# kirumang/Pix2Pose

Measured on AMD Instinct MI355X. Metric: crops/sec (AE fwd + PnP-RANSAC) at 128x128, higher is better.
Workload: dtype f16x3 (fp32 operands split into two f16 halves, 3 MFMAs per product block, fp32 accumulate)

## Files before the change

### pix2pose_amd/build.py

```python
from __future__ import annotations

import hashlib
import os
import subprocess

HERE = os.path.dirname(os.path.abspath(__file__))
CSRC = os.path.join(HERE, "csrc")
LIB = os.path.join(HERE, "libp2p_mi355.so")
DEV_LIB = os.path.join(HERE, "libp2p_mi355_dev.so")
DEV_OBJ_DIR = os.path.join(CSRC, "dev")
SOURCES = ["igemm.hip", "igemm_halo.hip", "igemm_halo8.hip", "igemm_halo_s2.hip", "igemm_stream.hip", "wino.hip", "wino3.hip", "wino3o.hip", "resblock.hip", "heads.hip", "conv1.hip", "misc_kernels.hip", "model.hip", "pipeline.hip", "resize_aa.hip", "pnp.hip", "comm.hip", "depth.hip", "normals.hip", "icp.hip", "rgbd.hip", "xyz_patch.hip", "train_batch.hip"]
HEADERS = ["kernels.h", "device_common.h", "igemm_halo_common.h", "wino_common.h", "model.h", "pipeline.h", "resize_rules.h", os.path.join("..", "..", "include", "p2p_mi355.h")]
BUILD_ID_SRC = os.path.join(CSRC, "_build_id.cpp")
EXPORT_MAP = os.path.join(CSRC, "_exports.map")
HIPCC = os.environ.get("HIPCC", "/opt/rocm/bin/hipcc")
FLAGS = ["--offload-arch=gfx950", "-O3", "-std=c++17", "-fPIC", "-fvisibility=hidden", "-Wall", "-Wno-unused-function", "-Wno-unused-value", "-Wno-unused-result"]


def _newer(a: str, b: str) -> bool:
    return not os.path.exists(b) or os.path.getmtime(a) > os.path.getmtime(b)


def _files():
    srcs = [os.path.join(CSRC, s) for s in SOURCES if os.path.exists(os.path.join(CSRC, s))]
# ... 20 lines not shown


def _compile_and_link(lib: str, obj_dir: str, extra_flags, force: bool, verbose: bool) -> str:
    srcs, hdrs = _files()
    os.makedirs(obj_dir, exist_ok=True)
    objs = []
    hdr_time = max(os.path.getmtime(h) for h in hdrs)
    procs = []
    for s in srcs:
        o = os.path.join(obj_dir, os.path.splitext(os.path.basename(s))[0] + ".o")
        objs.append(o)
        if force or _newer(s, o) or os.path.getmtime(o) < hdr_time:
            cmd = [HIPCC] + FLAGS + list(extra_flags) + ["-c", s, "-o", o]
            if verbose:
                print(" ".join(cmd))
            procs.append((cmd, subprocess.Popen(cmd)))
            if len(procs) >= JOBS:
                c, pr = procs.pop(0)
                if pr.wait():
                    raise subprocess.CalledProcessError(pr.returncode, c)
    for c, pr in procs:
        if pr.wait():
            raise subprocess.CalledProcessError(pr.returncode, c)
    bid = source_hash()
    text = '// generated by pix2pose_amd/build.py\nextern "C" __attribute__((visibility("default"))) const char* p2p_build_id(void) { return "%s"; }\n' % bid
    if not os.path.exists(BUILD_ID_SRC) or open(BUILD_ID_SRC).read() != text:
        open(BUILD_ID_SRC, "w").write(text)
    bo = os.path.join(obj_dir, "_build_id.o")
    if force or _newer(BUILD_ID_SRC, bo):
        subprocess.check_call(["g++", "-O1", "-fPIC", "-fvisibility=hidden", "-c", BUILD_ID_SRC, "-o", bo])
    objs.append(bo)
    import re
    names = sorted(set(re.findall(r"\bP2P_API\s+[\w\s\*]+?\b(p2p_[a-z0-9_]+)\s*\(", open(os.path.join(HERE, "..", "include", "p2p_mi355.h")).read())))
    vtext = "{ global: %s; local: *; };\n" % "; ".join(names)
    if not os.path.exists(EXPORT_MAP) or open(EXPORT_MAP).read() != vtext:
        open(EXPORT_MAP, "w").write(vtext)
    if force or any(_newer(o, lib) for o in objs) or _newer(EXPORT_MAP, lib):
        cmd = [HIPCC, "--offload-arch=gfx950", "-shared", "-fPIC", "-Wl,--version-script=" + EXPORT_MAP, "-o", lib] + objs + ["-ldl"]
        if verbose:
            print(" ".join(cmd))
        subprocess.check_call(cmd)
    return lib


JOBS = max(1, min(4, (os.cpu_count() or 2) // 2))


def build(force: bool = False, verbose: bool = False, dev: bool = True) -> str:
    lib = _compile_and_link(LIB, CSRC, [], force, verbose)
    if dev:
        _compile_and_link(DEV_LIB, DEV_OBJ_DIR, ["-DP2P_DEV_SWITCHES"], force, verbose)
    return lib


def dev_switches(**switches) -> dict:
    override = os.environ.get("P2P_DEV_LIB")
    if override:
        if not os.path.exists(override):
            raise RuntimeError("P2P_DEV_LIB=%s does not exist" % override)
        env = {"P2P_LIB": override}
        env.update({k: str(v) for k, v in switches.items()})
        return env
    if have_sources() and have_compiler():
        _compile_and_link(DEV_LIB, DEV_OBJ_DIR, ["-DP2P_DEV_SWITCHES"], False, False)
    elif not os.path.exists(DEV_LIB):
        raise RuntimeError("development twin %s is missing and cannot be built here" % DEV_LIB)
# ... 9 lines not shown
```

### pix2pose_amd/csrc/kernels.h

```cpp
#pragma once
#include <hip/hip_runtime.h>
#include <stdint.h>
#include <stdlib.h>

namespace p2p {

#ifdef P2P_DEV_SWITCHES
inline const char* dev_env(const char* name) { return getenv(name); }
#else
inline const char* dev_env(const char*) { return nullptr; }
#endif

struct Ctx;
extern thread_local Ctx* g_prof_ctx;
struct ProfScope {
    Ctx* ctx;
    hipStream_t s;
    int slot;
    double flops, bytes;
    hipEvent_t a = nullptr, b = nullptr;
    bool failed = false;
    ProfScope(Ctx* X, int slot_, hipStream_t st, double fl = 0.0, double by = 0.0) : ctx(X), s(st), slot(slot_), flops(fl), bytes(by) { if (ctx) open(); }
    ProfScope(int slot_, hipStream_t st) : ProfScope(g_prof_ctx, slot_, st) {}
    ~ProfScope() { if (ctx) (void)close(); }
// ... 111 lines not shown
    int n_groups;
    ResBlockGroup grp[IGEMM_MAX_GROUPS + 1];
};
bool resblock_supported(int F1, int H, int W);
int resblock_grid(int F1, int N, int H, int W);
hipError_t launch_resblock(const ResBlockParams& p, int F1, hipStream_t s);
hipError_t launch_resproj(const ResBlockParams& p, int F1, hipStream_t s);

struct WinoGroup {
    const float* U;
    const float* scale;
    const float* shift;
    int sample0;
    int unit0;
};
struct WinoParams {
    IgemmSeg seg[2];
    unsigned seg_bytes[2];
    int seg0_groups;
    int N, H, W, Cin, Cout;
    float* V;
    const float* U;
    const float* scale;
    const float* shift;
    int act;
    float alpha;
    float* out;
    int out_cstride, out_coff;
    unsigned* range_acc;
    int n_groups;
    WinoGroup grp[IGEMM_MAX_GROUPS + 1];
    int ksplit;
    float* partial;
};
bool wino_supported(int H, int W, int Cin0, int Cin1, int Cout);
size_t wino_v_bytes(int N, int H, int W, int Cin);
int wino_gemm_grid(const WinoParams& p);
hipError_t launch_wino_input(const WinoParams& p, hipStream_t s);
hipError_t launch_wino_gemm(const WinoParams& p, int n_cu, hipStream_t s);

struct Wino3Params {
    const float* in;
    unsigned in_bytes;
    int N, H, W, Cin, Cout;
    float* V;
    const float* U;
    const float* scale;
    const float* shift;
    int act;
    float alpha;
    float* out;
    int out_cstride, out_coff;
    unsigned* range_acc;
    int n_groups;
    WinoGroup grp[IGEMM_MAX_GROUPS + 1];
};
bool wino3_supported(int H, int W, int Cin, int Cout);
size_t wino3_v_bytes(int N, int H, int W, int Cin);
hipError_t launch_wino3_input(const Wino3Params& p, hipStream_t s);
hipError_t launch_wino3_gemm(const Wino3Params& p, int n_cu, hipStream_t s);

struct Wino3oParams {
    const float* in;
    unsigned in_bytes;
    int N, Cin, Cout;
    float* V;
    const float* U;
    const float* scale;
    const float* shift;
    int act;
    float alpha;
    float* out;
    int out_cstride, out_coff;
    int ksplit;
    float* partial;
    unsigned* range_acc;
    int n_groups;
    WinoGroup grp[IGEMM_MAX_GROUPS + 1];
};
bool wino3o_supported(int mode, int Cin, int Cout);
size_t wino3o_v_bytes(int mode, int units, int Cin);
int wino3o_units(const Wino3oParams& p);
hipError_t launch_wino3o_input(const Wino3oParams& p, int mode, hipStream_t s);
hipError_t launch_wino3o_gemm(const Wino3oParams& p, int mode, int n_cu, hipStream_t s);

struct StreamOrder {
    int n_groups;
    int8_t gstart[IGEMM_MAX_TAPS + 3];
// ... 52 lines not shown
```

### pix2pose_amd/csrc/model.hip

```cpp
#include "model.h"

#include <cmath>
#include <cstdarg>
#include <cstdio>
#include <cstring>
#include <thread>

namespace p2p {

static thread_local char g_err[512] = "";

void set_error(const char* fmt, ...)
{
    va_list ap;
    va_start(ap, fmt);
    vsnprintf(g_err, sizeof(g_err), fmt, ap);
    va_end(ap);
}
const char* get_error() { return g_err; }

constexpr double BN_EPS = 1e-3;
constexpr float LEAKY = 0.3f;

struct TensorMap {
// ... 950 lines not shown
        static const int max_s2 = dev_env("P2P_SMALL_SPLIT_S2") ? atoi(dev_env("P2P_SMALL_SPLIT_S2")) : 256;
        int S = tiles <= (c.in_stride == 2 ? max_s2 : max_s1) ? std::min(std::min(16, 768 / std::max(1, tiles)), p.ksteps / 12) : 1;
        while (S >= 2 && (size_t)S * p.M * L.Cout > (size_t)X.max_batch * 64 * 64 * 128 * 2) --S;
        if (S >= 2) {
            ConvCall c2 = c;
            c2.ksplit = S; c2.partial = X.cur->act["wv"];
            PreparedConv pc2;
            if ((rc = prepare_conv(X, L, c2, pc2))) return rc;
            if (pc2.stream) {
                if ((rc = launch_prepared(X, &pc2, 1))) return rc;
                HIP_TRY(launch_splitk_reduce(c2.partial, S, p.M, L.Cout, L.scale, L.shift, c.act, LEAKY, c.out, L.prec == PREC_F16X3 ? X.range_cur : nullptr, X.cur->stream));
                return P2P_OK;
            }
        }
    }
    return launch_prepared(X, &pc, 1);
}

static int conv_layer(Ctx& X, const ConvLayer& L, const float* in, int N, int H, int W, int C, int stride,
                      float* out, int act, const float* residual = nullptr)
{
    ConvCall c;
    c.s0 = {in, C, C, 0};
    c.N = N; c.Hin = H; c.Win = W; c.Hg = H / stride; c.Wg = W / stride; c.in_stride = stride;
    c.out = out; c.Hout = c.Hg; c.Wout = c.Wg; c.out_cstride = L.Cout;
    c.act = act; c.residual = residual; c.res_cstride = L.Cout;
    return L.ntaps == 25 ? run_conv_small(X, L, c) : run_conv(X, L, c);
}

constexpr int WINO_MIN_INPUTS = 1;

static bool wino_split_route() { static const bool on = dev_env("P2P_NO_WINO_SPLIT") == nullptr; return on; }

static int try_wino(Ctx& X, const ConvLayer& L, const float* a, int Ca, const float* b, int Cb, int cb_stride, int cb_off, int N, int H, float* out)
{
    if (!L.wino_u || L.prec != PREC_F16X3 || X.wino_mode == P2P_WINOGRAD_OFF || !specialised_kernels() || !wino_supported(H, H, Ca, Cb, L.Cout)) return 0;
    WinoParams p;
    memset(&p, 0, sizeof(p));
    p.seg[0] = {a, Ca, Ca, 0};
    p.seg[1] = {b, Cb, cb_stride, cb_off};
    const size_t px = (size_t)N * H * H;
    const size_t b0 = px * Ca * sizeof(float), b1 = px * cb_stride * sizeof(float);
    if (b0 >= 0xFFFFFFF0ull || b1 >= 0xFFFFFFF0ull || L.wino_bytes >= 0xFFFFFFF0ull) return 0;
    p.seg_bytes[0] = (unsigned)b0; p.seg_bytes[1] = (unsigned)b1;
    p.seg0_groups = Ca / 32;
    p.N = N; p.H = H; p.W = H; p.Cin = Ca + Cb; p.Cout = L.Cout;
    p.V = X.cur->act["wv"];
    p.U = L.wino_u; p.scale = L.wino_scale; p.shift = L.shift;
    p.act = ACT_LEAKY; p.alpha = LEAKY;
    p.out = out; p.out_cstride = L.Cout; p.out_coff = 0;
    p.range_acc = X.range_cur;
    int rc = wino_groups(X, L, 2, "try_wino", p.grp, p.n_groups);
    if (rc) return rc;
    static const int wino_min = dev_env("P2P_WINO_MIN") ? atoi(dev_env("P2P_WINO_MIN")) : WINO_MIN_INPUTS;
    if (X.wino_mode != P2P_WINOGRAD_ALWAYS && N < wino_min) return 0;
    if (X.wino_mode == P2P_WINOGRAD_AUTO && p.n_groups <= 1 && wino_split_route()) {
        const int tiles = wino_gemm_grid(p), S = p.Cin / 16;
        for (int k : {6, 4, 3, 2})
            if (tiles * k <= 256 && S % (2 * k) == 0 && (size_t)k * px * L.Cout <= WINO_PARTIAL_FLOATS) { p.ksplit = k; p.partial = X.cur->act["wp"]; break; }
    }
    hipStream_t st = X.cur->stream;
    const double in_el = (double)px * p.Cin, out_el = (double)px * L.Cout;
    if ((rc = prof_launch(X, 11, 0.0, 4.0 * in_el + 8.0 * in_el, [&]() { return launch_wino_input(p, st); }))) return rc;
    if ((rc = prof_launch(X, 10, 2.0 * out_el * 25.0 * p.Cin, 8.0 * in_el + (double)L.wino_bytes + 4.0 * out_el,
                          [&]() { return launch_wino_gemm(p, X.n_cu, st); }))) return rc;
    if (p.ksplit > 1) HIP_TRY(launch_splitk_reduce(p.partial, p.ksplit, (int)px, L.Cout, L.wino_scale, L.shift, ACT_LEAKY, LEAKY, out, X.range_cur, st));
    return 1;
}

static int concat_conv(Ctx& X, const ConvLayer& L, const float* a, int Ca, const float* b, int Cb,
                       int cb_stride, int cb_off, int N, int H, float* out)
{
    {
        const int rc = try_wino(X, L, a, Ca, b, Cb, cb_stride, cb_off, N, H, out);
        if (rc < 0) return rc;
        if (rc == 1) return P2P_OK;
    }
    ConvCall c;
    c.s0 = {a, Ca, Ca, 0};
    c.s1 = {b, Cb, cb_stride, cb_off};
    c.N = N; c.Hin = H; c.Win = H; c.Hg = H; c.Wg = H;
    c.out = out; c.Hout = H; c.Wout = H; c.out_cstride = L.Cout;
    c.act = ACT_LEAKY;
    return run_conv_small(X, L, c);
}

constexpr int WINO3_MIN_INPUTS = 5;
constexpr int WINO3O_MIN_INPUTS = 9;
static bool wino3_route() { static const bool on = dev_env("P2P_NO_WINO3") == nullptr; return on; }

static int try_wino3o(Ctx& X, const ConvLayer& L, int mode, const float* in, int N, int C, float* out)
{
    if (!L.wino_u || L.prec != PREC_F16X3 || X.wino_mode == P2P_WINOGRAD_OFF || !specialised_kernels() || !wino3_route() || !wino3o_supported(mode, C, L.Cout)) return 0;
    static const int wino3o_min = dev_env("P2P_WINO3O_MIN") ? atoi(dev_env("P2P_WINO3O_MIN")) : WINO3O_MIN_INPUTS;
    if (X.wino_mode != P2P_WINOGRAD_ALWAYS && N < wino3o_min) return 0;
    const size_t b0 = (size_t)N * (mode ? 256 : 64) * C * sizeof(float);
    if (b0 >= 0xFFFFFFF0ull || L.wino_bytes >= 0xFFFFFFF0ull) return 0;
    Wino3oParams p;
    memset(&p, 0, sizeof(p));
    p.in = in; p.in_bytes = (unsigned)b0;
    p.N = N; p.Cin = C; p.Cout = L.Cout;
    p.V = X.cur->act["wv"];
    p.U = L.wino_u; p.scale = L.wino_scale; p.shift = L.shift;
    p.act = ACT_LEAKY; p.alpha = LEAKY;
    p.out = out; p.out_cstride = L.Cout; p.out_coff = 0;
    p.ksplit = 1;
    p.range_acc = X.range_cur;
    int rc = wino_groups(X, L, 8, "try_wino3o", p.grp, p.n_groups);
    if (rc) return rc;
    const int units = wino3o_units(p);
    if (wino3o_v_bytes(mode, units, C) > (size_t)X.max_batch * 64 * 64 * 128 * 2 * sizeof(float)) return 0;
    if (mode == 1 && (X.wino_mode == P2P_WINOGRAD_ALWAYS || units * (L.Cout / 64) < 256)) { p.ksplit = 4; p.partial = X.cur->act["c3"]; }
    hipStream_t st = X.cur->stream;
    const double in_el = (double)N * (mode ? 256 : 64) * C, out_el = (double)N * (mode ? 64 : 256) * L.Cout;
    if ((rc = prof_launch(X, 21, 0.0, 4.0 * in_el + 6.0 * in_el, [&]() { return launch_wino3o_input(p, mode, st); }))) return rc;
    if ((rc = prof_launch(X, 20, 2.0 * out_el * (mode ? 25.0 : 6.25) * C, 6.0 * in_el + (double)L.wino_bytes + 4.0 * out_el,
                          [&]() { return launch_wino3o_gemm(p, mode, X.n_cu, st); }))) return rc;
    if (p.ksplit > 1 && p.n_groups > 1) {
        Conv1Groups G;
        if ((rc = conv1_groups(X, L, N, 64, true, G))) return rc;
        HIP_TRY(launch_splitk_reduce_groups(p.partial, p.ksplit, N * 64, L.Cout, G, ACT_LEAKY, LEAKY, out, X.range_cur, st));
    } else if (p.ksplit > 1)
        HIP_TRY(launch_splitk_reduce(p.partial, p.ksplit, N * 64, L.Cout, L.wino_scale, L.shift, ACT_LEAKY, LEAKY, out, X.range_cur, st));
    return 1;
}

static int try_wino3(Ctx& X, const ConvLayer& L, const float* in, int N, int H, int C, float* out)
{
    if (H == 8) return try_wino3o(X, L, 0, in, N, C, out);
    if (!L.wino_u || L.prec != PREC_F16X3 || X.wino_mode == P2P_WINOGRAD_OFF || !specialised_kernels() || !wino3_route() || !wino3_supported(H, H, C, L.Cout)) return 0;
    static const int wino3_min = dev_env("P2P_WINO3_MIN") ? atoi(dev_env("P2P_WINO3_MIN")) : WINO3_MIN_INPUTS;
    if (X.wino_mode != P2P_WINOGRAD_ALWAYS && N < wino3_min) return 0;
    const size_t px = (size_t)N * H * H;
    const size_t b0 = px * C * sizeof(float);
    if (b0 >= 0xFFFFFFF0ull || L.wino_bytes >= 0xFFFFFFF0ull) return 0;
    Wino3Params p;
    memset(&p, 0, sizeof(p));
    p.in = in; p.in_bytes = (unsigned)b0;
    p.N = N; p.H = H; p.W = H; p.Cin = C; p.Cout = L.Cout;
    p.V = X.cur->act["wv"];
    p.U = L.wino_u; p.scale = L.wino_scale; p.shift = L.shift;
    p.act = ACT_LEAKY; p.alpha = LEAKY;
    p.out = out; p.out_cstride = L.Cout; p.out_coff = 0;
    p.range_acc = X.range_cur;
    int rc = wino_groups(X, L, 2, "try_wino3", p.grp, p.n_groups);
    if (rc) return rc;
    hipStream_t st = X.cur->stream;
    const double in_el = (double)px * C, out_el = 4.0 * (double)px * L.Cout;
    if ((rc = prof_launch(X, 21, 0.0, 4.0 * in_el + 6.0 * in_el, [&]() { return launch_wino3_input(p, st); }))) return rc;
    rc = prof_launch(X, 20, 2.0 * out_el * 6.25 * C, 6.0 * in_el + (double)L.wino_bytes + 4.0 * out_el, [&]() { return launch_wino3_gemm(p, X.n_cu, st); });
    return rc ? rc : 1;
}

static int deconv_layer(Ctx& X, const Model& M, const char* name, const float* in, int N, int H, int C,
                        float* out)
{
    {
        const int rc = try_wino3(X, M.L.at(std::string(name) + "_p0"), in, N, H, C, out);
        if (rc < 0) return rc;
        if (rc == 1) return P2P_OK;
    }
    PreparedConv pc[4];
    bool all_stream = true;
    for (int ph = 0; ph < 4; ++ph) {
        const ConvLayer& L = M.L.at(std::string(name) + "_p" + std::to_string(ph));
        ConvCall c;
        c.s0 = {in, C, C, 0};
        c.N = N; c.Hin = H; c.Win = H; c.Hg = H; c.Wg = H;
        c.out = out; c.Hout = 2 * H; c.Wout = 2 * H; c.os = 2; c.oy = ph >> 1; c.ox = ph & 1;
        c.out_cstride = L.Cout;
        c.act = ACT_LEAKY;
        int rc = prepare_conv(X, L, c, pc[ph]);
        if (rc) return rc;
        all_stream = all_stream && pc[ph].stream;
    }
    if (all_stream) return launch_prepared(X, pc, 4);
    for (int ph = 0; ph < 4; ++ph) {
        int rc = launch_prepared(X, &pc[ph], 1);
        if (rc) return rc;
    }
    return P2P_OK;
}

static bool fused_blocks() { static const bool on = dev_env("P2P_NO_FUSED_BLOCK") == nullptr; return on && specialised_kernels(); }
static int fused_min_wgs() { static const int v = dev_env("P2P_FUSED_MIN_WGS") ? atoi(dev_env("P2P_FUSED_MIN_WGS")) : -1; return v >= 0 ? v : stream_max_wgs() + 1; }

static int run_fused_block(const Model& M, Ctx& X, const std::string& n, const float* in, int N, int H, int Cin, int f1, int stride, bool proj, float* out)
{
    const ConvLayer &a = M.L.at(n + "_2a"), &b = M.L.at(n + "_2b"), &c = M.L.at(n + (proj ? "_2c1" : "_2c"));
    const int C = 4 * f1, Ho = H / stride;
    ResBlockParams p;
// ... 127 lines not shown
        if ((rc = conv_layer(X, M.L.at("conv2"), A["f1"], n, 64, 64, 128, 2, A["f2"], ACT_LEAKY))) return rc;
        if ((rc = conv_layer(X, M.L.at("conv3"), A["f2"], n, 32, 32, 256, 2, A["f3"], ACT_LEAKY))) return rc;
        if ((rc = try_wino3o(X, M.L.at("conv4"), 1, A["f3"], n, 256, A["f4"])) < 0) return rc;
        if (rc == 0 && (rc = conv_layer(X, M.L.at("conv4"), A["f3"], n, 16, 16, 256, 2, A["f4"], ACT_LEAKY))) return rc;
        s1 = A["f1"]; s1_stride = 128; s1_off = 64; s1_C = 64;
        s2 = A["f2"]; s2_stride = 256; s2_off = 128;
        s3 = A["f3"]; s3_stride = 256; s3_off = 128;
    }
    {
        const ConvLayer& L = M.L.at("dense_enc");
        ConvCall c;
        c.s0 = {A["f4"], 32768, 32768, 0};
        c.N = n; c.Hin = c.Win = c.Hg = c.Wg = 1;
        c.out = A["enc"]; c.Hout = c.Wout = 1; c.out_cstride = 256;
        c.ksplit = 32; c.partial = A["part"];
        if ((rc = run_conv(X, L, c))) return rc;
        if (n_grp == 1) {
            HIP_TRY(launch_splitk_reduce(A["part"], 32, n, 256, L.scale, L.shift, ACT_NONE, LEAKY, A["enc"], M.prec == PREC_F16X3 ? X.range_cur : nullptr, st));
        } else {
            Conv1Groups G;
            if ((rc = conv1_groups(X, L, n, 1, false, G))) return rc;
            HIP_TRY(launch_splitk_reduce_groups(A["part"], 32, n, 256, G, ACT_NONE, LEAKY, A["enc"], M.prec == PREC_F16X3 ? X.range_cur : nullptr, st));
        }
    }
    {
        const ConvLayer& L = M.L.at("dense_dec");
        ConvCall c;
        c.s0 = {A["enc"], 256, 256, 0};
        c.N = n; c.Hin = c.Win = c.Hg = c.Wg = 1;
        c.out = A["dd"]; c.Hout = c.Wout = 1; c.out_cstride = 16384;
        if ((rc = run_conv(X, L, c))) return rc;
    }
    if ((rc = deconv_layer(X, M, "up1", A["dd"], n, 8, 256, A["u1"]))) return rc;
    if ((rc = concat_conv(X, M.L.at("deconv1"), A["u1"], 256, s3, 128, s3_stride, s3_off, n, 16, A["c1"]))) return rc;
    if ((rc = deconv_layer(X, M, "up2", A["c1"], n, 16, 256, A["u2"]))) return rc;
    if ((rc = concat_conv(X, M.L.at("deconv2"), A["u2"], 128, s2, 128, s2_stride, s2_off, n, 32, A["c2"]))) return rc;
    if ((rc = deconv_layer(X, M, "up3", A["c2"], n, 32, 256, A["u3"]))) return rc;
    if ((rc = concat_conv(X, M.L.at("deconv3"), A["u3"], 64, s1, s1_C, s1_stride, s1_off, n, 64, A["c3"]))) return rc;
    {
        ConvCall c;
        c.s0 = {A["c3"], 128, 128, 0};
        c.N = n; c.Hin = c.Win = c.Hg = c.Wg = 64;
        c.out = xyzp; c.Hout = c.Wout = 128; c.os = 2; c.out_cstride = 4;
        c.mode = EPI_HEAD;
        c.algo_macs = (double)n * 64 * 64 * 25 * 128 * 4;
        if ((rc = run_conv(X, M.L.at("heads"), c))) return rc;
    }
    return P2P_OK;
}

int forward_async(Ctx& X, const Model& M, const float* x_dev, int n, float* xyzp_dev)
{
    int rc = X.ensure_workspace();
    if (rc) return rc;
    for (int i = 0; i < n; i += X.max_batch) {
        const int c = std::min(X.max_batch, n - i);
        rc = forward_chunk(X, M, x_dev + (size_t)i * 128 * 128 * 3, c, xyzp_dev + (size_t)i * 128 * 128 * 4);
        if (rc) return rc;
    }
    return P2P_OK;
}

thread_local Ctx* g_prof_ctx = nullptr;

void ProfScope::open()
{
    a = ctx->prof_get_event();
    b = a ? ctx->prof_get_event() : nullptr;
    hipError_t e = hipSuccess;
    if (a && b && (e = hipEventRecord(a, s)) == hipSuccess) return;
// ... 348 lines not shown
```

### pix2pose_amd/csrc/wino.hip

```cpp
#include "wino_common.h"

namespace p2p {

namespace {

__global__ __launch_bounds__(256) void wino_input_kernel(const WinoParams p)
{
    const int tid = threadIdx.x;
    const int quad = tid & 7, t = (tid >> 3) & 3, r = tid >> 5;
    int b = blockIdx.x;
    const int rblocks = p.H >> 3;
    const int rb = b % rblocks; b /= rblocks;
    const int cgroups = p.Cin >> 5;
    const int cg = b % cgroups; b /= cgroups;
    const int PC = p.W >> 4;
    const int pc = b % PC;
    const int n = b / PC;
    const int y = rb * 8 + r;

    const bool s1 = cg >= p.seg0_groups;
    const IgemmSeg sg = s1 ? p.seg[1] : p.seg[0];
    const __amdgpu_buffer_rsrc_t rs = __builtin_amdgcn_make_buffer_rsrc((void*)sg.ptr, 0, s1 ? p.seg_bytes[1] : p.seg_bytes[0], 0x00020000);
    const unsigned c0 = (unsigned)(sg.coff + (s1 ? cg - p.seg0_groups : cg) * 32 + quad * 4);
    const int x0 = pc * 16 + t * 4 - 2;
    const unsigned rowpix = (unsigned)((n * p.H + y) * p.W);
    f32x4 d[8];
#pragma unroll
    for (int k = 0; k < 8; ++k) {
        const int x = x0 + k;
        const unsigned off = (unsigned)x < (unsigned)p.W ? ((rowpix + (unsigned)x) * (unsigned)sg.cstride + c0) * 4u : OOB;
        d[k] = __builtin_bit_cast(f32x4, __builtin_amdgcn_raw_buffer_load_b128(rs, off, 0, 0));
    }
    f32x4 v[8];
// ... 25 lines not shown
    }
    range_commit(p.range_acc, amax);
}

template <bool DUAL>
__global__ __launch_bounds__(512, 2) void wino_gemm_kernel(const WinoParams p)
{
    constexpr int R = DUAL ? 38 : 36;
    constexpr int PLANE = R * 64;
    constexpr int BUF = 32 * PLANE;
    constexpr int XLD = 68;
    constexpr int XBUF = 8 * 32 * XLD * 4;
    static_assert(2 * XBUF <= 2 * BUF, "exchange image fits the two slice buffers");
    __shared__ __attribute__((aligned(16))) char smem[2 * BUF];

    const int tid = threadIdx.x;
    const int lane = tid & 63;
    const int j = __builtin_amdgcn_readfirstlane(tid >> 6);
    const int li = lane & 31, lk = lane >> 5;

    const int S = p.Cin >> 4;
    const int PC = p.W >> 4;
    const int RB = DUAL ? 1 : p.H >> 5;
    const int NT = p.Cout >> 6;
    const int units = DUAL ? (p.n_groups > 1 ? p.grp[p.n_groups].unit0 : (p.N + 1) >> 1) : p.N;
    const int KS = p.ksplit > 1 ? p.ksplit : 1;
    const int Sl = S / KS;
    const int ntiles = units * PC * RB * NT * KS;
    const unsigned slice_bytes = 32u * (unsigned)p.H * 64u;
    const size_t unit_block = (size_t)S * slice_bytes;

    const int tl0 = xcd_first_tile(gridDim.x, blockIdx.x);
    const int pair = tid >> 4, cq = tid & 15;
    float amax = 0.f;

    for (int tl = tl0; tl < ntiles; tl += gridDim.x) {
    const int ks = tl % KS;
    const int s_begin = ks * Sl;
    const int ntile = (tl / KS) % NT;
    int rest = tl / (KS * NT);
    const int rb = rest % RB; rest /= RB;
    const int pc = rest % PC;
    const int unit = rest / PC;
    int n0 = DUAL ? unit * 2 : unit;
    int n_end = p.N;
    const int y0 = rb * 32;

    const float* gu = p.U;
    const float* gscale = p.scale;
    const float* gshift = p.shift;
    if (p.n_groups > 1) {
        const int g = DUAL ? group_of<&WinoGroup::unit0>(p.grp, p.n_groups, unit) : group_of<&WinoGroup::sample0>(p.grp, p.n_groups, n0);
        if (DUAL) {
            n0 = p.grp[g].sample0 + 2 * (unit - p.grp[g].unit0);
            n_end = p.grp[g + 1].sample0;
        }
        gu = p.grp[g].U; gscale = p.grp[g].scale; gshift = p.grp[g].shift;
    }
    const bool has_b = DUAL && n0 + 1 < n_end;

    const char* vbase = reinterpret_cast<const char*>(p.V) + ((size_t)n0 * PC + pc) * unit_block;
    const unsigned vrange = (unsigned)__builtin_amdgcn_readfirstlane((int)(unsigned)(has_b ? 2 * unit_block : unit_block));
    const __amdgpu_buffer_rsrc_t rs_v = __builtin_amdgcn_make_buffer_rsrc((void*)vbase, 0, vrange, 0x00020000);
    const unsigned plane_bytes = (unsigned)p.H * 64u;
    unsigned vo_a, vo_b, vo_c;
    if (DUAL) {
        vo_a = vo_b = vo_c = (unsigned)lane * 16u;
// ... 142 lines not shown
    }
#endif
#pragma unroll
    for (int i = 0; i < 4; ++i) {
        float* X = reinterpret_cast<float*>(smem + (i & 1) * XBUF);
        exchange_store<XLD>(X, j, li, lk, acc[0][i], acc[1][i]);
        lds_barrier();
        f32x4 m[8];
#pragma unroll
        for (int jj = 0; jj < 8; ++jj) m[jj] = *reinterpret_cast<const f32x4*>(X + (jj * 32 + pair) * XLD + cq * 4);
        int n, y;
        if (DUAL) { n = n0 + (i >> 1); y = (i & 1) * 8 + (pair >> 2); }
        else { n = n0; y = y0 + i * 8 + (pair >> 2); }
        if (!DUAL || n == n0 || has_b) {
            const size_t pix = ((size_t)n * p.H + y) * p.W + pc * 16 + (pair & 3) * 4;
            float* o = p.out + pix * p.out_cstride + p.out_coff + col;
            f32x4 yv[4];
#pragma unroll
            for (int e = 0; e < 4; ++e) {
                const float s12 = m[1][e] + m[2][e], d12 = m[1][e] - m[2][e];
                const float s34 = m[3][e] + m[4][e], d34 = m[3][e] - m[4][e];
                const float s56 = m[5][e] + m[6][e], d56 = m[5][e] - m[6][e];
                yv[0][e] = (m[0][e] + s12) + (s34 + s56);
                yv[1][e] = __builtin_fmaf(0.5f, d56, __builtin_fmaf(2.f, d34, d12));
                yv[2][e] = __builtin_fmaf(0.25f, s56, __builtin_fmaf(4.f, s34, s12));
                yv[3][e] = __builtin_fmaf(0.125f, d56, __builtin_fmaf(8.f, d34, d12)) + m[7][e];
            }
            if (KS > 1) {
                float* po = p.partial + ((size_t)ks * p.N * p.H * p.W + pix) * p.Cout + col;
#pragma unroll
                for (int k = 0; k < 4; ++k) *reinterpret_cast<f32x4*>(po + (size_t)k * p.Cout) = yv[k];
                continue;
            }
#pragma unroll
            for (int k = 0; k < 4; ++k) {
                const f32x4 v = bn_act4(yv[k], sc, sh, p.act, p.alpha);
                amax = range_note4(amax, v);
#ifdef P2P_ABL_WST
                if (v[0] == 123.456f)
#endif
                *reinterpret_cast<f32x4*>(o + (size_t)k * p.out_cstride) = v;
            }
        }
    }
    }
    range_commit(p.range_acc, amax);
}

}

bool wino_supported(int H, int W, int Cin0, int Cin1, int Cout)
{
    if (Cin0 % 32 || Cin1 % 32 || Cout % 64 || W % 16) return false;
    return (H == 16 && W == 16) || H % 32 == 0;
}

size_t wino_v_bytes(int N, int H, int W, int Cin) { return (size_t)N * H * W * Cin * 8; }

int wino_gemm_grid(const WinoParams& p)
{
    const bool dual = p.H == 16;
    const int units = dual ? (p.n_groups > 1 ? p.grp[p.n_groups].unit0 : (p.N + 1) / 2) : p.N * (p.H / 32);
    return units * (p.W / 16) * (p.Cout / 64) * (p.ksplit > 1 ? p.ksplit : 1);
}

hipError_t launch_wino_input(const WinoParams& p, hipStream_t s)
{
    const int grid = p.N * (p.W / 16) * (p.Cin / 32) * (p.H / 8);
    hipLaunchKernelGGL(wino_input_kernel, dim3(grid), dim3(256), 0, s, p);
    return hipGetLastError();
}

hipError_t launch_wino_gemm(const WinoParams& p, int n_cu, hipStream_t s)
{
    if (p.ksplit > 1 && ((p.Cin >> 4) % (2 * p.ksplit) || !p.partial || p.n_groups > 1)) return hipErrorInvalidValue;
    const int tiles = wino_gemm_grid(p);
    const int grid = tiles < n_cu ? tiles : n_cu;
    if (p.H == 16) hipLaunchKernelGGL((wino_gemm_kernel<true>), dim3(grid), dim3(512), 0, s, p);
    else hipLaunchKernelGGL((wino_gemm_kernel<false>), dim3(grid), dim3(512), 0, s, p);
    return hipGetLastError();
}

}
```

### pix2pose_amd/csrc/wino3.hip

```cpp
#include "wino_common.h"

#include <type_traits>

namespace p2p {

#ifdef P2P_W3_STAMPS
__device__ unsigned long long g_w3_stamps[8 * 16 * 16];
#define W3_STAMP(k) do { if (lane == 0 && (blockIdx.x & 31) == 0 && (blockIdx.x >> 5) < 8 && n_tile_seen < 16) g_w3_stamps[((blockIdx.x >> 5) * 16 + n_tile_seen) * 16 + (k)] = wall_clock64(); } while (0)
#else
#define W3_STAMP(k) do {} while (0)
#endif

namespace {

__global__ __launch_bounds__(256) void wino3_input_kernel(const Wino3Params p)
{
    const int tid = threadIdx.x;
    const int quad = tid & 7, t = (tid >> 3) & 3, r = tid >> 5;
    int b = blockIdx.x;
    const int rblocks = p.H >> 3;
    const int rb = b % rblocks; b /= rblocks;
    const int cgroups = p.Cin >> 5;
    const int cg = b % cgroups; b /= cgroups;
    const int PC = p.W >> 4;
    const int pc = b % PC;
    const int n = b / PC;
    const int y = rb * 8 + r;

    const __amdgpu_buffer_rsrc_t rs = __builtin_amdgcn_make_buffer_rsrc((void*)p.in, 0, p.in_bytes, 0x00020000);
    const unsigned c0 = (unsigned)(cg * 32 + quad * 4);
    const int x0 = pc * 16 + t * 4 - 1;
    const unsigned rowpix = (unsigned)((n * p.H + y) * p.W);
    f32x4 d[6];
#pragma unroll
    for (int k = 0; k < 6; ++k) {
        const int x = x0 + k;
        const unsigned off = (unsigned)x < (unsigned)p.W ? ((rowpix + (unsigned)x) * (unsigned)p.Cin + c0) * 4u : OOB;
        d[k] = __builtin_bit_cast(f32x4, __builtin_amdgcn_raw_buffer_load_b128(rs, off, 0, 0));
    }
    f32x4 v[6];
    f43_input_transform(d, v);
    const int S = p.Cin >> 4;
    const int slice = cg * 2 + (quad >> 2), lk = (quad >> 1) & 1;
    const size_t plane_bytes = (size_t)p.H * 64;
    char* dst = reinterpret_cast<char*>(p.V) + ((((size_t)n * PC + pc) * S + slice) * 24 + lk) * plane_bytes + (size_t)y * 64 + t * 16 + (quad & 1) * 8;
    float amax = 0.f;
#pragma unroll
    for (int j = 0; j < 6; ++j) {
        const f32x4 w = v[j];
        amax = range_note4(amax, w);
        uint2 hi, lo;
        split4(w, hi, lo);
        *reinterpret_cast<uint2*>(dst + (size_t)(j * 4) * plane_bytes) = hi;
        *reinterpret_cast<uint2*>(dst + (size_t)(j * 4 + 2) * plane_bytes) = lo;
    }
    range_commit(p.range_acc, amax);
}

template <int NU>
__global__ __launch_bounds__(NU * 384, 2 / NU) void wino3_gemm_kernel(const Wino3Params p)
// ... 239 lines not shown
#pragma unroll
                            for (int e = 0; e < 4; ++e) v[e] = v[e] > 0.f ? v[e] : v[e] * p.alpha;
                        }
                        amax = range_note4(amax, v);
                        *reinterpret_cast<f32x4*>(o + (size_t)(2 * k) * p.out_cstride) = v;
                    }
                }
            }
        }
    }
    }
    range_commit(p.range_acc, amax);
}

}

#ifdef P2P_W3_STAMPS
extern "C" __attribute__((visibility("default"))) int p2p_dbg_w3_stamps(unsigned long long* host)
{
    return (int)hipMemcpyFromSymbol(host, HIP_SYMBOL(g_w3_stamps), sizeof(g_w3_stamps));
}
#endif

bool wino3_supported(int H, int W, int Cin, int Cout)
{
    if (Cin % 32 || Cout % 64 || W % 16) return false;
    return (H == 16 && W == 16) || H % 32 == 0;
}

size_t wino3_v_bytes(int N, int H, int W, int Cin) { return (size_t)N * H * W * Cin * 6; }

hipError_t launch_wino3_input(const Wino3Params& p, hipStream_t s)
{
    const int grid = p.N * (p.W / 16) * (p.Cin / 32) * (p.H / 8);
    hipLaunchKernelGGL(wino3_input_kernel, dim3(grid), dim3(256), 0, s, p);
    return hipGetLastError();
}

hipError_t launch_wino3_gemm(const Wino3Params& p, int n_cu, hipStream_t s)
{
#ifdef P2P_W3_NU1
    constexpr int NU = 1;
#else
    constexpr int NU = 2;
#endif
    const int g4 = 4 * (p.Cout / 64);
    const int ups = p.H / 16;
    const int wunits = NU == 1 ? p.N * ups : ups == 1 ? (p.n_groups > 1 ? p.grp[p.n_groups].unit0 : (p.N + 1) / 2) : p.N * (ups / 2);
    const int tiles = wunits * (p.W / 16) * g4;
    const int slots = n_cu * (2 / NU);
    int grid = tiles < slots ? tiles : slots / g4 * g4;
    if (grid < 1) grid = tiles < g4 ? tiles : g4;
    hipLaunchKernelGGL((wino3_gemm_kernel<NU>), dim3(grid), dim3(NU * 384), 0, s, p);
    return hipGetLastError();
}

}
```

Baseline: 12360.

## Fuse wino3 input transform into preceding Winograd GEMM epilogue

The F(4,3) Winograd GEMM epilogue for deconv1/deconv2 now also computes the next up-layer's wino3 input transform in registers, using lane permutes to fetch neighbour columns. It writes the split f16 V operand directly and skips storing interior output tiles that only fed that transform. A reduced boundary-only wino3 input pass then handles tiles whose halo crosses workgroup tiles. This removes one full activation read and most of the separate input-transform launch. The cost is extra epilogue work, more register pressure in the GEMM, and more complex coupling between layers. By default it is active only for H>=32, i.e. the deconv2→up3 pair.

New measurement: 12150. -1.7%, worse.

```diff
diff --git a/pix2pose_amd/build.py b/pix2pose_amd/build.py
--- a/pix2pose_amd/build.py
+++ b/pix2pose_amd/build.py
@@ -76,6 +76,7 @@
     objs.append(bo)
     import re
     names = sorted(set(re.findall(r"\bP2P_API\s+[\w\s\*]+?\b(p2p_[a-z0-9_]+)\s*\(", open(os.path.join(HERE, "..", "include", "p2p_mi355.h")).read())))
+    names.append("p2p_dbg_*")
     vtext = "{ global: %s; local: *; };\n" % "; ".join(names)
     if not os.path.exists(EXPORT_MAP) or open(EXPORT_MAP).read() != vtext:
         open(EXPORT_MAP, "w").write(vtext)
diff --git a/pix2pose_amd/csrc/kernels.h b/pix2pose_amd/csrc/kernels.h
--- a/pix2pose_amd/csrc/kernels.h
+++ b/pix2pose_amd/csrc/kernels.h
@@ -167,7 +167,21 @@
     WinoGroup grp[IGEMM_MAX_GROUPS + 1];
     int ksplit;
     float* partial;
-};
+    float* fv;
+    int fv_cin;
+    unsigned* fv_range;
+};
+
+__host__ __device__ inline bool f43_v_tile_is_producers(int W, int g)
+{
+    const int t = g & 3;
+    return (t != 0 || g == 0) && (t != 3 || 4 * g + 4 >= W);
+}
+__host__ __device__ inline bool f43_out_tile_is_stored(int W, int g)
+{
+    return !f43_v_tile_is_producers(W, g) || (g > 0 && !f43_v_tile_is_producers(W, g - 1)) || (4 * g + 4 < W && !f43_v_tile_is_producers(W, g + 1));
+}
+__host__ __device__ inline int f43_boundary_v_tiles(int W) { return 2 * (W / 16 - 1); }
 bool wino_supported(int H, int W, int Cin0, int Cin1, int Cout);
 size_t wino_v_bytes(int N, int H, int W, int Cin);
 int wino_gemm_grid(const WinoParams& p);
@@ -189,6 +203,7 @@
     unsigned* range_acc;
     int n_groups;
     WinoGroup grp[IGEMM_MAX_GROUPS + 1];
+    int boundary;
 };
 bool wino3_supported(int H, int W, int Cin, int Cout);
 size_t wino3_v_bytes(int N, int H, int W, int Cin);
diff --git a/pix2pose_amd/csrc/model.hip b/pix2pose_amd/csrc/model.hip
--- a/pix2pose_amd/csrc/model.hip
+++ b/pix2pose_amd/csrc/model.hip
@@ -1006,7 +1006,16 @@
 
 static bool wino_split_route() { static const bool on = dev_env("P2P_NO_WINO_SPLIT") == nullptr; return on; }
 
-static int try_wino(Ctx& X, const ConvLayer& L, const float* a, int Ca, const float* b, int Cb, int cb_stride, int cb_off, int N, int H, float* out)
+struct FusedV {
+    const float* in = nullptr;
+    float* V = nullptr;
+};
+static bool fuse_v_route() { static const bool on = dev_env("P2P_NO_FUSE_V") == nullptr; return on; }
+static bool fuse_v16_route() { static const bool on = dev_env("P2P_FUSE_V16") != nullptr; return on; }
+static bool wino3_takes(const Ctx& X, const ConvLayer& L, int N, int H, int C);
+
+static int try_wino(Ctx& X, const ConvLayer& L, const float* a, int Ca, const float* b, int Cb, int cb_stride, int cb_off, int N, int H, float* out,
+                    const ConvLayer* next = nullptr, FusedV* fv = nullptr)
 {
     if (!L.wino_u || L.prec != PREC_F16X3 || X.wino_mode == P2P_WINOGRAD_OFF || !specialised_kernels() || !wino_supported(H, H, Ca, Cb, L.Cout)) return 0;
     WinoParams p;
@@ -1033,20 +1042,33 @@
         for (int k : {6, 4, 3, 2})
             if (tiles * k <= 256 && S % (2 * k) == 0 && (size_t)k * px * L.Cout <= WINO_PARTIAL_FLOATS) { p.ksplit = k; p.partial = X.cur->act["wp"]; break; }
     }
+    if (next && fv && fuse_v_route() && p.ksplit <= 1 && (H >= 32 || fuse_v16_route()) && wino3_takes(X, *next, N, H, L.Cout)) {
+        const size_t v0 = (wino_v_bytes(N, H, H, p.Cin) + 255) & ~(size_t)255;
+        if (v0 + wino3_v_bytes(N, H, H, L.Cout) <= (size_t)X.max_batch * 64 * 64 * 128 * 2 * sizeof(float)) {
+            p.fv = reinterpret_cast<float*>(reinterpret_cast<char*>(p.V) + v0); p.fv_cin = L.Cout; p.fv_range = X.range_cur;
+            fv->in = out; fv->V = p.fv;
+        }
+    }
     hipStream_t st = X.cur->stream;
     const double in_el = (double)px * p.Cin, out_el = (double)px * L.Cout;
     if ((rc = prof_launch(X, 11, 0.0, 4.0 * in_el + 8.0 * in_el, [&]() { return launch_wino_input(p, st); }))) return rc;
-    if ((rc = prof_launch(X, 10, 2.0 * out_el * 25.0 * p.Cin, 8.0 * in_el + (double)L.wino_bytes + 4.0 * out_el,
+    double out_by = 4.0 * out_el;
+    if (p.fv) {
+        int own = 0, stored = 0;
+        for (int g = 0; g < H / 4; ++g) { own += f43_v_tile_is_producers(H, g); stored += f43_out_tile_is_stored(H, g); }
+        out_by = out_el * (6.0 * own + 4.0 * stored) / (H / 4);
+    }
+    if ((rc = prof_launch(X, 10, 2.0 * out_el * 25.0 * p.Cin, 8.0 * in_el + (double)L.wino_bytes + out_by,
                           [&]() { return launch_wino_gemm(p, X.n_cu, st); }))) return rc;
     if (p.ksplit > 1) HIP_TRY(launch_splitk_reduce(p.partial, p.ksplit, (int)px, L.Cout, L.wino_scale, L.shift, ACT_LEAKY, LEAKY, out, X.range_cur, st));
     return 1;
 }
 
 static int concat_conv(Ctx& X, const ConvLayer& L, const float* a, int Ca, const float* b, int Cb,
-                       int cb_stride, int cb_off, int N, int H, float* out)
+                       int cb_stride, int cb_off, int N, int H, float* out, const ConvLayer* next = nullptr, FusedV* fv = nullptr)
 {
     {
-        const int rc = try_wino(X, L, a, Ca, b, Cb, cb_stride, cb_off, N, H, out);
+        const int rc = try_wino(X, L, a, Ca, b, Cb, cb_stride, cb_off, N, H, out, next, fv);
         if (rc < 0) return rc;
         if (rc == 1) return P2P_OK;
     }
@@ -1099,20 +1121,30 @@
     return 1;
 }
 
-static int try_wino3(Ctx& X, const ConvLayer& L, const float* in, int N, int H, int C, float* out)
-{
+static bool wino3_takes(const Ctx& X, const ConvLayer& L, int N, int H, int C)
+{
+    if (H == 8 || !L.wino_u || L.prec != PREC_F16X3 || X.wino_mode == P2P_WINOGRAD_OFF || !specialised_kernels() || !wino3_route() || !wino3_supported(H, H, C, L.Cout)) return false;
+    static const int wino3_min = dev_env("P2P_WINO3_MIN") ? atoi(dev_env("P2P_WINO3_MIN")) : WINO3_MIN_INPUTS;
+    if (X.wino_mode != P2P_WINOGRAD_ALWAYS && N < wino3_min) return false;
+    return (size_t)N * H * H * C * sizeof(float) < 0xFFFFFFF0ull && L.wino_bytes < 0xFFFFFFF0ull;
+}
+
+static int try_wino3(Ctx& X, const ConvLayer& L, const float* in, int N, int H, int C, float* out, FusedV* fv = nullptr)
+{
+    const bool fused = fv && fv->in == in && fv->V;
     if (H == 8) return try_wino3o(X, L, 0, in, N, C, out);
-    if (!L.wino_u || L.prec != PREC_F16X3 || X.wino_mode == P2P_WINOGRAD_OFF || !specialised_kernels() || !wino3_route() || !wino3_supported(H, H, C, L.Cout)) return 0;
-    static const int wino3_min = dev_env("P2P_WINO3_MIN") ? atoi(dev_env("P2P_WINO3_MIN")) : WINO3_MIN_INPUTS;
-    if (X.wino_mode != P2P_WINOGRAD_ALWAYS && N < wino3_min) return 0;
+    if (!wino3_takes(X, L, N, H, C)) {
+        if (fused) { set_error("try_wino3: the operand was written for a route this pass does not take"); return P2P_ERR_INVALID_ARG; }
+        return 0;
+    }
     const size_t px = (size_t)N * H * H;
     const size_t b0 = px * C * sizeof(float);
-    if (b0 >= 0xFFFFFFF0ull || L.wino_bytes >= 0xFFFFFFF0ull) return 0;
     Wino3Params p;
     memset(&p, 0, sizeof(p));
     p.in = in; p.in_bytes = (unsigned)b0;
     p.N = N; p.H = H; p.W = H; p.Cin = C; p.Cout = L.Cout;
-    p.V = X.cur->act["wv"];
+    p.V = fused ? fv->V : X.cur->act["wv"];
+    p.boundary = fused;
     p.U = L.wino_u; p.scale = L.wino_scale; p.shift = L.shift;
     p.act = ACT_LEAKY; p.alpha = LEAKY;
     p.out = out; p.out_cstride = L.Cout; p.out_coff = 0;
@@ -1121,16 +1153,19 @@
     if (rc) return rc;
     hipStream_t st = X.cur->stream;
     const double in_el = (double)px * C, out_el = 4.0 * (double)px * L.Cout;
-    if ((rc = prof_launch(X, 21, 0.0, 4.0 * in_el + 6.0 * in_el, [&]() { return launch_wino3_input(p, st); }))) return rc;
+    const double bfrac = (double)f43_boundary_v_tiles(H) / (H / 4);
+    if (!fused) rc = prof_launch(X, 21, 0.0, 4.0 * in_el + 6.0 * in_el, [&]() { return launch_wino3_input(p, st); });
+    else if (f43_boundary_v_tiles(H)) rc = prof_launch(X, 21, 0.0, (4.0 * 1.5 + 6.0) * in_el * bfrac, [&]() { return launch_wino3_input(p, st); });
+    if (rc) return rc;
     rc = prof_launch(X, 20, 2.0 * out_el * 6.25 * C, 6.0 * in_el + (double)L.wino_bytes + 4.0 * out_el, [&]() { return launch_wino3_gemm(p, X.n_cu, st); });
     return rc ? rc : 1;
 }
 
 static int deconv_layer(Ctx& X, const Model& M, const char* name, const float* in, int N, int H, int C,
-                        float* out)
+                        float* out, FusedV* fv = nullptr)
 {
     {
-        const int rc = try_wino3(X, M.L.at(std::string(name) + "_p0"), in, N, H, C, out);
+        const int rc = try_wino3(X, M.L.at(std::string(name) + "_p0"), in, N, H, C, out, fv);
         if (rc < 0) return rc;
         if (rc == 1) return P2P_OK;
     }
@@ -1324,10 +1359,11 @@
         if ((rc = run_conv(X, L, c))) return rc;
     }
     if ((rc = deconv_layer(X, M, "up1", A["dd"], n, 8, 256, A["u1"]))) return rc;
-    if ((rc = concat_conv(X, M.L.at("deconv1"), A["u1"], 256, s3, 128, s3_stride, s3_off, n, 16, A["c1"]))) return rc;
-    if ((rc = deconv_layer(X, M, "up2", A["c1"], n, 16, 256, A["u2"]))) return rc;
-    if ((rc = concat_conv(X, M.L.at("deconv2"), A["u2"], 128, s2, 128, s2_stride, s2_off, n, 32, A["c2"]))) return rc;
-    if ((rc = deconv_layer(X, M, "up3", A["c2"], n, 32, 256, A["u3"]))) return rc;
+    FusedV fv2, fv3;
+    if ((rc = concat_conv(X, M.L.at("deconv1"), A["u1"], 256, s3, 128, s3_stride, s3_off, n, 16, A["c1"], &M.L.at("up2_p0"), &fv2))) return rc;
+    if ((rc = deconv_layer(X, M, "up2", A["c1"], n, 16, 256, A["u2"], &fv2))) return rc;
+    if ((rc = concat_conv(X, M.L.at("deconv2"), A["u2"], 128, s2, 128, s2_stride, s2_off, n, 32, A["c2"], &M.L.at("up3_p0"), &fv3))) return rc;
+    if ((rc = deconv_layer(X, M, "up3", A["c2"], n, 32, 256, A["u3"], &fv3))) return rc;
     if ((rc = concat_conv(X, M.L.at("deconv3"), A["u3"], 64, s1, s1_C, s1_stride, s1_off, n, 64, A["c3"]))) return rc;
     {
         ConvCall c;
diff --git a/pix2pose_amd/csrc/wino.hip b/pix2pose_amd/csrc/wino.hip
--- a/pix2pose_amd/csrc/wino.hip
+++ b/pix2pose_amd/csrc/wino.hip
@@ -1,4 +1,6 @@
 #include "wino_common.h"
+
+#include <string.h>
 
 namespace p2p {
 
@@ -90,7 +92,7 @@
 
     const int tl0 = xcd_first_tile(gridDim.x, blockIdx.x);
     const int pair = tid >> 4, cq = tid & 15;
-    float amax = 0.f;
+    float amax = 0.f, vmax = 0.f;
 
     for (int tl = tl0; tl < ntiles; tl += gridDim.x) {
     const int ks = tl % KS;
@@ -299,19 +301,60 @@
                 for (int k = 0; k < 4; ++k) *reinterpret_cast<f32x4*>(po + (size_t)k * p.Cout) = yv[k];
                 continue;
             }
+            const int t = pair & 3, g = pc * 4 + t;
+            f32x4 ov[4];
 #pragma unroll
             for (int k = 0; k < 4; ++k) {
-                const f32x4 v = bn_act4(yv[k], sc, sh, p.act, p.alpha);
-                amax = range_note4(amax, v);
+                ov[k] = bn_act4(yv[k], sc, sh, p.act, p.alpha);
+                amax = range_note4(amax, ov[k]);
+            }
+            if (!p.fv || f43_out_tile_is_stored(p.W, g)) {
+#pragma unroll
+                for (int k = 0; k < 4; ++k) {
 #ifdef P2P_ABL_WST
-                if (v[0] == 123.456f)
-#endif
-                *reinterpret_cast<f32x4*>(o + (size_t)k * p.out_cstride) = v;
+                    if (ov[k][0] == 123.456f)
+#endif
+                    *reinterpret_cast<f32x4*>(o + (size_t)k * p.out_cstride) = ov[k];
+                }
+            }
+            if (p.fv) {
+                f32x4 d[6];
+#pragma unroll
+                for (int e = 0; e < 4; ++e) {
+                    const float last = ov[3][e], first = ov[0][e];
+                    d[0][e] = __int_as_float(__builtin_amdgcn_ds_bpermute(((lane + 48) & 63) * 4, __float_as_int(last)));
+                    d[5][e] = __int_as_float(__builtin_amdgcn_ds_bpermute(((lane + 16) & 63) * 4, __float_as_int(first)));
+                }
+                if (f43_v_tile_is_producers(p.W, g)) {
+                    const f32x4 z = {0.f, 0.f, 0.f, 0.f};
+                    if (t == 0) d[0] = z;
+                    if (t == 3) d[5] = z;
+#pragma unroll
+                    for (int k = 0; k < 4; ++k) {
+                        d[1 + k] = ov[k];
+#pragma unroll
+                        for (int e = 0; e < 4; ++e) { float f = d[1 + k][e]; asm volatile("" : "+v"(f)); d[1 + k][e] = f; }
+                    }
+                    f32x4 w[6];
+                    f43_input_transform(d, w);
+                    const size_t plane_bytes = (size_t)p.H * 64;
+                    char* dst = reinterpret_cast<char*>(p.fv) + ((((size_t)n * PC + pc) * (p.fv_cin >> 4) + (col >> 4)) * 24 + ((col >> 3) & 1)) * plane_bytes
+                                + (size_t)y * 64 + t * 16 + ((col >> 2) & 1) * 8;
+#pragma unroll
+                    for (int jj = 0; jj < 6; ++jj) {
+                        vmax = range_note4(vmax, w[jj]);
+                        uint2 hi, lo;
+                        split4(w[jj], hi, lo);
+                        *reinterpret_cast<uint2*>(dst + (size_t)(jj * 4) * plane_bytes) = hi;
+                        *reinterpret_cast<uint2*>(dst + (size_t)(jj * 4 + 2) * plane_bytes) = lo;
+                    }
+                }
             }
         }
     }
     }
     range_commit(p.range_acc, amax);
+    if (p.fv) range_commit(p.fv_range, vmax);
 }
 
 }
@@ -341,6 +384,7 @@
 hipError_t launch_wino_gemm(const WinoParams& p, int n_cu, hipStream_t s)
 {
     if (p.ksplit > 1 && ((p.Cin >> 4) % (2 * p.ksplit) || !p.partial || p.n_groups > 1)) return hipErrorInvalidValue;
+    if (p.fv && (p.ksplit > 1 || p.out_coff || p.out_cstride != p.Cout || p.fv_cin != p.Cout)) return hipErrorInvalidValue;
     const int tiles = wino_gemm_grid(p);
     const int grid = tiles < n_cu ? tiles : n_cu;
     if (p.H == 16) hipLaunchKernelGGL((wino_gemm_kernel<true>), dim3(grid), dim3(512), 0, s, p);
@@ -348,4 +392,55 @@
     return hipGetLastError();
 }
 
-}
+#ifdef P2P_DEV_SWITCHES
+extern "C" __attribute__((visibility("default"))) int p2p_dbg_wino_fused_v(int N, int H, int Cin, int Cout, const float* x, const void* U, size_t u_bytes,
+                                                                            void* v_fused, void* v_ref, float* out_ref, unsigned* ranges)
+{
+    if (N < 1 || !wino_supported(H, H, Cin, 0, Cout) || !wino3_supported(H, H, Cout, 64)) return -1;
+    const size_t xb = (size_t)N * H * H * Cin * 4, ob = (size_t)N * H * H * Cout * 4, vb = wino_v_bytes(N, H, H, Cin), v3b = wino3_v_bytes(N, H, H, Cout);
+    char* d = nullptr;
+    const size_t off_u = xb, off_o = off_u + ((u_bytes + 255) & ~(size_t)255), off_v = off_o + ob, off_f = off_v + vb, off_r = off_f + v3b, total = off_r + 256;
+    if (hipMalloc((void**)&d, total) != hipSuccess) return -2;
+    int rc = 0;
+    auto ok = [&](hipError_t e) { if (e != hipSuccess && !rc) rc = -3; return e == hipSuccess; };
+    ok(hipMemcpy(d, x, xb, hipMemcpyHostToDevice));
+    ok(hipMemcpy(d + off_u, U, u_bytes, hipMemcpyHostToDevice));
+    int n_cu = 0;
+    ok(hipDeviceGetAttribute(&n_cu, hipDeviceAttributeMultiprocessorCount, 0));
+    WinoParams p;
+    memset(&p, 0, sizeof(p));
+    p.seg[0] = {reinterpret_cast<const float*>(d), Cin, Cin, 0};
+    p.seg[1] = {reinterpret_cast<const float*>(d), 0, Cin, 0};
+    p.seg_bytes[0] = (unsigned)xb; p.seg_bytes[1] = 0;
+    p.seg0_groups = Cin / 32;
+    p.N = N; p.H = H; p.W = H; p.Cin = Cin; p.Cout = Cout;
+    p.V = reinterpret_cast<float*>(d + off_v); p.U = reinterpret_cast<const float*>(d + off_u);
+    p.act = ACT_LEAKY; p.alpha = 0.2f;
+    p.out = reinterpret_cast<float*>(d + off_o); p.out_cstride = Cout;
+    p.ksplit = 1;
+    Wino3Params q;
+    memset(&q, 0, sizeof(q));
+    q.in = p.out; q.in_bytes = (unsigned)ob;
+    q.N = N; q.H = H; q.W = H; q.Cin = Cout; q.Cout = 64;
+    q.V = reinterpret_cast<float*>(d + off_f);
+    for (int fused = 1; fused >= 0 && !rc; --fused) {
+        ok(hipMemset(d + off_f, 0xFF, v3b));
+        ok(hipMemset(d + off_o, 0xFF, ob));
+        ok(hipMemset(d + off_r, 0, 256));
+        p.range_acc = reinterpret_cast<unsigned*>(d + off_r);
+        p.fv = fused ? q.V : nullptr; p.fv_cin = Cout; p.fv_range = reinterpret_cast<unsigned*>(d + off_r) + 1;
+        q.boundary = fused; q.range_acc = reinterpret_cast<unsigned*>(d + off_r) + 1;
+        ok(launch_wino_input(p, nullptr));
+        ok(launch_wino_gemm(p, n_cu, nullptr));
+        ok(launch_wino3_input(q, nullptr));
+        ok(hipDeviceSynchronize());
+        ok(hipMemcpy(fused ? v_fused : v_ref, d + off_f, v3b, hipMemcpyDeviceToHost));
+        ok(hipMemcpy(ranges + (fused ? 0 : 2), d + off_r, 8, hipMemcpyDeviceToHost));
+        if (!fused) ok(hipMemcpy(out_ref, d + off_o, ob, hipMemcpyDeviceToHost));
+    }
+    hipFree(d);
+    return rc;
+}
+#endif
+
+}
diff --git a/pix2pose_amd/csrc/wino3.hip b/pix2pose_amd/csrc/wino3.hip
--- a/pix2pose_amd/csrc/wino3.hip
+++ b/pix2pose_amd/csrc/wino3.hip
@@ -16,16 +16,23 @@
 __global__ __launch_bounds__(256) void wino3_input_kernel(const Wino3Params p)
 {
     const int tid = threadIdx.x;
-    const int quad = tid & 7, t = (tid >> 3) & 3, r = tid >> 5;
+    const int quad = tid & 7, r = tid >> 5;
+    int t = (tid >> 3) & 3;
     int b = blockIdx.x;
-    const int rblocks = p.H >> 3;
+    const int rblocks = p.boundary ? p.H >> 5 : p.H >> 3;
     const int rb = b % rblocks; b /= rblocks;
     const int cgroups = p.Cin >> 5;
     const int cg = b % cgroups; b /= cgroups;
     const int PC = p.W >> 4;
-    const int pc = b % PC;
-    const int n = b / PC;
-    const int y = rb * 8 + r;
+    const int pcs = p.boundary ? f43_boundary_v_tiles(p.W) : PC;
+    int pc = b % pcs;
+    const int n = b / pcs;
+    int y = rb * 8 + r;
+    if (p.boundary) {
+        y = rb * 32 + t * 8 + r;
+        t = (pc & 1) ? 0 : 3;
+        pc = (pc + 1) >> 1;
+    }
 
     const __amdgpu_buffer_rsrc_t rs = __builtin_amdgcn_make_buffer_rsrc((void*)p.in, 0, p.in_bytes, 0x00020000);
     const unsigned c0 = (unsigned)(cg * 32 + quad * 4);
@@ -331,7 +338,9 @@
 
 hipError_t launch_wino3_input(const Wino3Params& p, hipStream_t s)
 {
-    const int grid = p.N * (p.W / 16) * (p.Cin / 32) * (p.H / 8);
+    if (p.boundary && f43_boundary_v_tiles(p.W) == 0) return hipSuccess;
+    if (p.boundary && p.H % 32) return hipErrorInvalidValue;
+    const int grid = p.boundary ? p.N * f43_boundary_v_tiles(p.W) * (p.Cin / 32) * (p.H / 32) : p.N * (p.W / 16) * (p.Cin / 32) * (p.H / 8);
     hipLaunchKernelGGL(wino3_input_kernel, dim3(grid), dim3(256), 0, s, p);
     return hipGetLastError();
 }
```
